# imalexlee/simple-vk-renderer

Hardware: AMD Instinct MI355X
Metric: shaded fragments/s (higher is better)
Workload: dtype f32

## Files before the change

simple-vk-renderer_amd/csrc/k_tile.hip:

```cpp
#include <hip/hip_ext.h>

#include <cstdlib>
#include <type_traits>

#include "svr_launch.h"
#include "svr_pixel.h"

namespace svr {

constexpr uint32_t REC_COMMON = 0x80000000u;
#ifndef SVR_PRIO_COST
#define SVR_PRIO_COST 200u
#endif
constexpr int BATCH = 64;
constexpr uint32_t SREC = 7;

constexpr float kG0 = 0x1.c51282p-2f, kG1 = -0x1.14a3a2p-2f, kG2 = 0x1.37536ap-3f, kG3 = -0x1.778474p-5f;

__device__ __forceinline__ float lod_from_rho2(float rho2) {
  uint32_t bits = f2u(rho2);
  int e = (int)(bits >> 23) - 127;
  float m = u2f((bits & 0x7fffffu) | 0x3f800000u);
  float t = m - 1.0f;
  float g = fmaf(fmaf(fmaf(kG3, t, kG2), t, kG1), t, kG0);
  float s = t * (1.0f - t);
  float l = fmaf(s, g, t);
  float lam = 0.5f * ((float)e + l);
  lam = (rho2 <= 0x1p+100f) ? lam : 50.0f;
  lam = (rho2 >= 0x1p-100f) ? lam : -50.0f;
  return lam;
}

__device__ __forceinline__ float lerpf(float a, float b, float t) { return fmaf(t, b - a, a); }

struct TexD {
  uint32_t base_off;
  uint32_t w, h, lw, lh, levels, filters;
  float min_lod, max_lod;
};

struct Taps {
  uint32_t o00, o10, o01, o11;
  float alpha, beta;
};
template <bool POW2 = false>
__device__ __forceinline__ Taps level_taps(int wl, int hl, uint32_t plw, uint32_t base, bool linear, float u, float v) {
  float U = (u - floorf(u)) * (float)wl;
  float V = (v - floorf(v)) * (float)hl;
  float Uh = U - 0.5f, Vh = V - 0.5f;
  float fu = floorf(linear ? Uh : U), fv = floorf(linear ? Vh : V);
  Taps tp;
  tp.alpha = linear ? Uh - fu : 0.0f;
  tp.beta = linear ? Vh - fv : 0.0f;
  int i0 = (int)fu, j0 = (int)fv;
  int i1 = linear ? i0 + 1 : i0, j1 = linear ? j0 + 1 : j0;
  if (POW2) {
    i0 &= wl - 1;
    i1 &= wl - 1;
    j0 &= hl - 1;
    j1 &= hl - 1;
  } else {
    if (i0 < 0) i0 += wl;
    if (i0 >= wl) i0 -= wl;
    if (i1 >= wl) i1 -= wl;
    if (j0 < 0) j0 += hl;
    if (j0 >= hl) j0 -= hl;
    if (j1 >= hl) j1 -= hl;
  }
  const uint32_t x0 = texel_offset_x((uint32_t)i0), x1 = texel_offset_x((uint32_t)i1);
  const uint32_t y0 = base + texel_offset_y(plw, (uint32_t)j0), y1 = base + texel_offset_y(plw, (uint32_t)j1);
  tp.o00 = y0 + x0;
  tp.o10 = y0 + x1;
  tp.o01 = y1 + x0;
  tp.o11 = y1 + x1;
  return tp;
}
__device__ __forceinline__ uint32_t texel(const uint8_t* arena, uint32_t off) {
  return *reinterpret_cast<const uint32_t*>(arena + off);
}
__device__ __forceinline__ float bilerp(uint32_t t00, uint32_t t10, uint32_t t01, uint32_t t11, int c, float a, float b) {
  return lerpf(lerpf(chan(t00, c), chan(t10, c), a), lerpf(chan(t01, c), chan(t11, c), a), b);
}

__device__ __forceinline__ float interp3(float a0, float da1, float da2, float b1, float b2, float r) {
  return fmaf(b2, da2, fmaf(b1, da1, a0)) * r;
}

struct FragAttr {
  float b1, b2, r, u, v, nx, ny, nz, light, cr, cg, cb, won;
};

__device__ __forceinline__ float quad_partner_x(float v) { return u2f((uint32_t)__builtin_amdgcn_mov_dpp((int)f2u(v), 0xB1, 0xf, 0xf, true)); }
__device__ __forceinline__ float quad_partner_y(float v) { return u2f((uint32_t)__builtin_amdgcn_mov_dpp((int)f2u(v), 0x128, 0xf, 0xf, true)); }
template <bool TRACE, bool COMMON = false, bool ATTR = false>
__device__ __forceinline__ float4 shade_pixel(const FrameParams& P, uint32_t rec, int px, int py, float* trace, const bool quads = false,
                                              FragAttr* fa = nullptr) {
  const TriRec* tr = P.recs + rec;
  const uint4* q4 = reinterpret_cast<const uint4*>(tr);
  const float4* f4 = reinterpret_cast<const float4*>(tr);
  const double2* d2 = reinterpret_cast<const double2*>(tr);
  uint4 hdr = q4[0];
  float4 zrow = f4[1];
  double2 c2 = d2[2], c3 = d2[3], c4 = d2[4], c5 = d2[5], c6 = d2[6];
  uint4 td = q4[7];
  float4 s0 = f4[8], s1 = f4[9], s2 = f4[10], s3 = f4[11], s4 = f4[12], s5 = f4[13], s6 = f4[14];
  uint32_t flags = hdr.w;
  float inv_area = zrow.w;
  double A1, B1, A2, B2, e1, e2;
  double C1 = c5.y, C2 = c6.x;
  A1 = c2.y; B1 = c4.x; A2 = c3.x; B2 = c4.y;
  double dx = (double)px, dy = (double)py;
  e1 = fma(A1, dx, fma(B1, dy, C1)) + ((flags & F_T1) ? 1.0 : 0.0);
  e2 = fma(A2, dx, fma(B2, dy, C2)) + ((flags & F_T2) ? 1.0 : 0.0);
  TexD t;
  t.base_off = (uint32_t)(unsigned long long)__double_as_longlong(c6.y);
  const uint32_t tk = (uint32_t)((unsigned long long)__double_as_longlong(c6.y) >> 32);
  t.w = td.x & 0xffffu;
  t.h = td.x >> 16;
  t.lw = td.y & 0xffu;
  t.lh = (td.y >> 8) & 0xffu;
  t.levels = (td.y >> 16) & 0xffu;
  t.filters = td.y >> 24;
  t.min_lod = u2f(td.z);
  t.max_lod = u2f(td.w);
  float b1 = (float)e1 * inv_area, b2 = (float)e2 * inv_area;
  float q0 = s0.x, dq1 = s0.y, dq2 = s0.z;
  const float qq = fmaf(b2, dq2, fmaf(b1, dq1, q0));
  float hb1 = 0.0f, hb2 = 0.0f, vb1 = 0.0f, vb2 = 0.0f, hq = 1.0f, vq = 1.0f, hr = 0.0f, vr = 0.0f;
  auto partners = [&]() {
    double sxp = (px & 1) ? -1.0 : 1.0, syp = (py & 1) ? -1.0 : 1.0;
    hb1 = (float)fma(sxp, A1, e1) * inv_area, hb2 = (float)fma(sxp, A2, e2) * inv_area;
    vb1 = (float)fma(syp, B1, e1) * inv_area, vb2 = (float)fma(syp, B2, e2) * inv_area;
    hq = fmaf(hb2, dq2, fmaf(hb1, dq1, q0)), vq = fmaf(vb2, dq2, fmaf(vb1, dq1, q0));
  };
  if (!COMMON && !quads) partners();
  const float r = COMMON ? rcp_in_window(qq) : rcp_ieee(qq);
  const uint32_t kind = COMMON ? (uint32_t)PIPE_MESH : ((flags >> F_KIND_SHIFT) & 3u);
  float cr = interp3(s1.z, s3.z, s5.z, b1, b2, r);
  float cg = interp3(s1.w, s3.w, s5.w, b1, b2, r);
  float cb = interp3(s2.x, s4.x, s6.x, b1, b2, r);
  if (ATTR) { fa->b1 = b1; fa->b2 = b2; fa->r = r; fa->won = 1.0f; }
  if (kind == PIPE_COLORED_TRIANGLE) return make_float4(cr, cg, cb, 1.0f);
  float u = interp3(s2.y, s4.y, s6.y, b1, b2, r), v = interp3(s2.z, s4.z, s6.z, b1, b2, r);
  if (ATTR) { fa->u = u; fa->v = v; }
  if (!COMMON) {
    hr = rcp_ieee(hq);
    vr = rcp_ieee(vq);
  }
  float uh, vh, uv_, vv_;
  if (quads) {
    uh = quad_partner_x(u), vh = quad_partner_x(v);
    uv_ = quad_partner_y(u), vv_ = quad_partner_y(v);
  } else {
    if (COMMON) {
      partners();
      hr = rcp_in_window(hq);
      vr = rcp_in_window(vq);
    }
    uh = interp3(s2.y, s4.y, s6.y, hb1, hb2, hr), vh = interp3(s2.z, s4.z, s6.z, hb1, hb2, hr);
    uv_ = interp3(s2.y, s4.y, s6.y, vb1, vb2, vr), vv_ = interp3(s2.z, s4.z, s6.z, vb1, vb2, vr);
  }
  float dudx = (px & 1) ? (u - uh) : (uh - u);
  float dvdx = (px & 1) ? (v - vh) : (vh - v);
  float dudy = (py & 1) ? (u - uv_) : (uv_ - u);
  float dvdy = (py & 1) ? (v - vv_) : (vv_ - v);
  float W0 = (float)t.w, H0 = (float)t.h;
  float mx = dudx * W0, my = dvdx * H0;
  float nx_ = dudy * W0, ny_ = dvdy * H0;
  float rho2 = fmaxf(fmaf(mx, mx, my * my), fmaf(nx_, nx_, ny_ * ny_));
  float lambda = fminf(fmaxf(lod_from_rho2(rho2), t.min_lod), t.max_lod);
  const bool linear = COMMON ? true : (((lambda <= 0.0f) ? (t.filters & 1u) : ((t.filters >> 1) & 1u)) != 0u);
  int q = COMMON ? (int)(tk >> 24) : (int)t.levels - 1;
  const bool mip_linear = COMMON ? true : (((t.filters >> 2) & 1u) != 0u);
  int dn = min(max((int)ceilf(lambda + 0.5f) - 1, 0), q);
  float lc = fminf(fmaxf(lambda, 0.0f), (float)q);
  float fl = floorf(lc);
  int dhi = mip_linear ? (int)fl : dn;
  float delta = mip_linear ? lc - fl : 0.0f;
  int dlo = mip_linear ? min(dhi + 1, q) : dn;
  float us = (COMMON || fabsf(u) < 8388608.0f) ? u : 0.0f, vs = (COMMON || fabsf(v) < 8388608.0f) ? v : 0.0f;
  const int whi = (int)max(t.w >> dhi, 1u), hhi = (int)max(t.h >> dhi, 1u);
  const uint32_t bhi = t.base_off + (COMMON ? packed_mip_offset(tk, (uint32_t)dhi) : mip_offset(t.lw, t.lh, (uint32_t)dhi));
  const uint32_t plw_hi = COMMON ? packed_level_lw(td.y, (uint32_t)dhi) : level_lw(t.lw, (uint32_t)dhi);
  Taps th = level_taps<COMMON>(whi, hhi, plw_hi, bhi, linear, us, vs);
  const uint8_t* tb = P.tex_arena;
  uint32_t h00 = texel(tb, th.o00), h10 = texel(tb, th.o10), h01 = texel(tb, th.o01), h11 = texel(tb, th.o11);
  const bool two_levels = __any(delta != 0.0f);
  Taps tl = th;
  uint32_t l00 = 0, l10 = 0, l01 = 0, l11 = 0;
  if (two_levels) {
    const int wlo = (int)max(t.w >> dlo, 1u), hlo = (int)max(t.h >> dlo, 1u);
    const uint32_t step = COMMON ? packed_level_bytes(tk, (uint32_t)dhi) : level_bytes(t.lw, t.lh, (uint32_t)dhi);
    const uint32_t blo = dlo != dhi ? bhi + step : bhi;
    const uint32_t plw_lo = COMMON ? packed_level_lw(td.y, (uint32_t)dlo) : level_lw(t.lw, (uint32_t)dlo);
    tl = level_taps<COMMON>(wlo, hlo, plw_lo, blo, linear, us, vs);
    l00 = texel(tb, tl.o00);
    l10 = texel(tb, tl.o10);
    l01 = texel(tb, tl.o01);
    l11 = texel(tb, tl.o11);
  }
  float4 tx;
  tx.x = bilerp(h00, h10, h01, h11, 0, th.alpha, th.beta);
  tx.y = bilerp(h00, h10, h01, h11, 1, th.alpha, th.beta);
  tx.z = bilerp(h00, h10, h01, h11, 2, th.alpha, th.beta);
  tx.w = 1.0f;
  if (two_levels) {
    tx.x = lerpf(tx.x, bilerp(l00, l10, l01, l11, 0, tl.alpha, tl.beta), delta);
    tx.y = lerpf(tx.y, bilerp(l00, l10, l01, l11, 1, tl.alpha, tl.beta), delta);
    tx.z = lerpf(tx.z, bilerp(l00, l10, l01, l11, 2, tl.alpha, tl.beta), delta);
  }
  if (TRACE) {
    trace[0] = (float)(hdr.z >> 2); trace[1] = b1; trace[2] = b2; trace[3] = r; trace[4] = u; trace[5] = v;
    trace[6] = dudx; trace[7] = dvdx; trace[8] = dudy; trace[9] = dvdy; trace[10] = lambda;
    trace[11] = tx.x; trace[12] = tx.y; trace[13] = tx.z;
    trace[26] = hb1; trace[27] = hb2; trace[28] = vb1; trace[29] = vb2; trace[30] = hr; trace[31] = vr;
  }
  if (kind == PIPE_TEX_IMAGE) {
    tx.w = bilerp(h00, h10, h01, h11, 3, th.alpha, th.beta);
    if (two_levels) tx.w = lerpf(tx.w, bilerp(l00, l10, l01, l11, 3, tl.alpha, tl.beta), delta);
    return tx;
  }
  float nx = interp3(s0.w, s2.w, s4.w, b1, b2, r);
  float ny = interp3(s1.x, s3.x, s5.x, b1, b2, r);
  float nz = interp3(s1.y, s3.y, s5.y, b1, b2, r);
  const float* L = P.scene.sunlight_direction;
  float d = fmaf(nz, L[2], fmaf(ny, L[1], nx * L[0]));
  float light = fmaxf(d, 0.1f);
  float sunw = P.scene.sunlight_color[3];
  cr = cr * tx.x;
  cg = cg * tx.y;
  cb = cb * tx.z;
  float4 o;
  o.x = fmaf(cr * light, sunw, cr * P.scene.ambient_color[0]);
  o.y = fmaf(cg * light, sunw, cg * P.scene.ambient_color[1]);
  o.z = fmaf(cb * light, sunw, cb * P.scene.ambient_color[2]);
  o.w = 1.0f;
  if (TRACE) {
    trace[15] = nx; trace[16] = ny; trace[17] = nz; trace[18] = cr; trace[19] = cg; trace[20] = cb;
    trace[21] = light; trace[22] = o.x; trace[23] = o.y; trace[24] = o.z; trace[25] = o.w;
  }
  if (ATTR) { fa->nx = nx; fa->ny = ny; fa->nz = nz; fa->light = light; fa->cr = cr; fa->cg = cg; fa->cb = cb; }
  return o;
}

template <bool INSTR, bool LIST, bool HIZ>
__device__ __forceinline__ void scan_columns(const FrameParams& P, uint4* s_cov, const uint32_t* s_list, uint32_t bin_base, uint32_t n,
                                             unsigned long long* s_depth, uint32_t* s_bm, int tx0, int ty0, int ry0, int nrows,
                                             uint32_t& n_raster, uint32_t& n_hiz_bad, uint32_t& occl) {
  auto entry = [&](uint32_t i) -> uint32_t { return LIST ? (s_list[i] & 0x7fffffffu) : P.bins[bin_base + i]; };
  const uint32_t lane = threadIdx.x & 63u, wave = threadIdx.x >> 6;
  static_assert(BATCH * 8 == 512, "two pieces per thread");
  uint4 pre0 = make_uint4(0, 0, 0, 0), pre1 = pre0;
  {
    uint32_t cnt = min((uint32_t)BATCH, n);
    const bool staged = (threadIdx.x & 7u) < SREC;
    if (staged && threadIdx.x < cnt * 8u) pre0 = reinterpret_cast<const uint4*>(P.recs + entry(threadIdx.x >> 3))[threadIdx.x & 7u];
    if (staged && threadIdx.x + 256u < cnt * 8u) pre1 = reinterpret_cast<const uint4*>(P.recs + entry(32u + (threadIdx.x >> 3)))[threadIdx.x & 7u];
  }
  constexpr uint32_t SVR_HIZ_MIN = BATCH;
  constexpr uint32_t SVR_HIZ_KEEP_COLS = 192u;
  const bool hiz = HIZ && n > (uint32_t)SVR_HIZ_MIN;
  uint32_t cur = 0, hz_cols = 0, hz_batches = 0, hz_pause = 0;
  if (hiz && threadIdx.x < 32u) s_bm[threadIdx.x] = threadIdx.x < 16u ? 0u : 0xffffffffu;
  for (uint32_t b0 = 0; b0 < n; b0 += BATCH) {
    uint32_t cnt = min((uint32_t)BATCH, n - b0);
    __syncthreads();
    const bool test = hiz && b0 && hz_pause == 0u;
    if (hiz && b0 && hz_pause) hz_pause--;
    if (test) {
      cur ^= 1u;
      const uint32_t b = threadIdx.x >> 4, k = threadIdx.x & 15u;
      const uint4* c4 = reinterpret_cast<const uint4*>(s_depth + ((b & 3u) * 8u + (k >> 1)) * TILE + (b >> 2) * 8u + (k & 1u) * 4u);
      const uint4 lo = c4[0], hi = c4[1];
// ... 79 lines not shown
          m = min(m, (by0 <= 3 && by1 >= 3) ? q.w : 0xffffffffu);
        }
        hidden = zb < m;
        if (hidden) gone = (uint32_t)cw;
        if (!INSTR && hidden) cw = 0;
      }
      if (INSTR && cw) {
        uint32_t* fl = reinterpret_cast<uint32_t*>(s_cov) + lane * SREC * 4u + 3u;
        *fl = (*fl & 0x7fffffffu) | ((hidden || (LIST && (s_list[b0 + lane] >> 31))) ? 0x80000000u : 0u);
      }
    }
    if (test) {
      const uint32_t nh = (uint32_t)__popcll(__ballot(hidden));
      hz_cols += nh + 3u * (uint32_t)__popcll(__ballot(gone >= 4u)) + 12u * (uint32_t)__popcll(__ballot(gone >= 16u));
      if (++hz_batches == 2u) {
        if (hz_cols < SVR_HIZ_KEEP_COLS) hz_pause = 6u;
        hz_cols = hz_batches = 0u;
      }
    }
    uint32_t inc = (uint32_t)cw;
#pragma unroll
    for (int off = 1; off < 64; off <<= 1) {
      uint32_t v = __shfl_up(inc, off);
      if ((int)lane >= off) inc += v;
    }
    uint32_t total = (uint32_t)__builtin_amdgcn_readlane((int)inc, 63);
    const uint32_t sh = total <= 64u ? 2u : (total <= 128u ? 1u : 0u);
    const int band_rows = nrows >> sh;
    const uint32_t items = total << sh;
    for (uint32_t c = wave; c * 64u < items; c += 4u) {
      uint32_t item = c * 64u + lane;
      uint32_t j = item >> sh, band = item & ((1u << sh) - 1u);
      bool act = item < items;
      uint32_t pos = 0;
#pragma unroll
      for (uint32_t step = 32; step >= 1; step >>= 1) {
        uint32_t v = __shfl(inc, (int)min(pos + step - 1u, 63u));
        if (pos + step <= 64u && v <= j) pos += step;
      }
      uint32_t i = min(pos, 63u);
      uint32_t excl = __shfl(inc, (int)i) - (uint32_t)__shfl(cw, (int)i);
      int col = __shfl(cx0, (int)i) + (int)(j - excl);
      if (!act) continue;
      const uint4* rec = s_cov + i * SREC;
      uint4 h = rec[0];
      int miny = (int)(int16_t)(h.x >> 16), maxy = (int)(int16_t)(h.y >> 16);
      int y0 = max(miny, ry0 + (int)band * band_rows), y1 = min(maxy, ry0 + (int)band * band_rows + band_rows - 1);
      if (y0 > y1) continue;
      uint32_t key = h.z, flags = h.w;
      float4 zr = reinterpret_cast<const float4*>(rec)[1];
      const double2* d = reinterpret_cast<const double2*>(rec);
      double2 c2 = d[2], c3 = d[3], c4 = d[4], c5 = d[5], c6 = d[6];
      double B0 = c3.y, B1 = c4.x, B2 = c4.y;
      double u1 = (flags & F_T1) ? 1.0 : 0.0, u2 = (flags & F_T2) ? 1.0 : 0.0;
      double dx = (double)col, dy = (double)y0;
      double f0 = fma(c2.x, dx, fma(B0, dy, c5.x));
      double f1 = fma(c2.y, dx, fma(B1, dy, c5.y));
      double f2 = fma(c3.x, dx, fma(B2, dy, c6.x));
      unsigned long long* cell = s_depth + (y0 - ty0) * TILE + (col - tx0);
      for (int y = y0; y <= y1; y++) {
        if (f0 >= 0.0 && f1 >= 0.0 && f2 >= 0.0) {
          if (INSTR) n_raster++;
          float b1 = (float)(f1 + u1) * zr.w, b2 = (float)(f2 + u2) * zr.w;
          float z = fmaf(b2, zr.z, fmaf(b1, zr.y, zr.x));
          z = fminf(fmaxf(z, 0.0f), 1.0f) + 0.0f;
          if (INSTR && (flags >> 31) && f2u(z) >= (uint32_t)(*cell >> 32)) n_hiz_bad++;
          atomicMax(cell, ((unsigned long long)f2u(z) << 32) | key);
        }
        f0 += B0;
        f1 += B1;
        f2 += B2;
        cell += TILE;
      }
    }
  }
}

__device__ __forceinline__ uint32_t resolve_record(const FrameParams& P, uint32_t rec, int px, int py) {
  uint4 h = *reinterpret_cast<const uint4*>(P.recs + rec);
  if ((int)(int16_t)(h.x & 0xffffu) <= (int)(int16_t)(h.y & 0xffffu)) return rec;
  double dx = (double)px, dy = (double)py;
  for (uint32_t c = 0; c < h.w; c++) {
    const TriRec* t = P.recs + h.z + c;
    if (t->minx > t->maxx || px < t->minx || px > t->maxx || py < t->miny || py > t->maxy) continue;
    if (fma(t->A[0], dx, fma(t->B[0], dy, t->C[0])) >= 0.0 && fma(t->A[1], dx, fma(t->B[1], dy, t->C[1])) >= 0.0 &&
        fma(t->A[2], dx, fma(t->B[2], dy, t->C[2])) >= 0.0)
      return h.z + c;
  }
  return rec;
}

constexpr uint32_t SORT_CAP = SPLIT_SORT_MAX;
constexpr uint32_t RANK_SORT_MAX = 1024;
#ifndef SVR_HIZ_FILTER_MIN
#define SVR_HIZ_FILTER_MIN 1024
#endif
constexpr uint32_t HIZ_AVG_ENTRIES = 96;
constexpr uint32_t HIZ_FILTER_MIN = SVR_HIZ_FILTER_MIN;
constexpr uint32_t QUARTER_LIST_CAP = 3808;
constexpr uint32_t QUEUE_CAP = 128;

template <int FMT, bool INSTR>
__device__ __forceinline__ void flush_fragments(const FrameParams& P, typename Codec<FMT>::enc_t* col, uint2* q,
                                                float4* s_src, uint32_t& qn, int tx0, int by0,
                                                uint32_t lane, uint32_t& n_shaded) {
  typedef Codec<FMT> CD;
  uint32_t cnt = min(qn, 64u);
// ... 84 lines not shown
      if (t0 < cnt) {
        if (pc < SREC) s_cov[t0 * SREC + pc] = r0;
        if (pc == 0) s_idx[t0] = ri0;
      }
      if (t0 + 32u < cnt) {
        if (pc < SREC) s_cov[(t0 + 32u) * SREC + pc] = r1;
        if (pc == 0) s_idx[t0 + 32u] = ri1;
      }
    }
    __syncthreads();
    int cx0 = 0, cw = 0;
    if (lane < cnt) {
      uint4 h = s_cov[lane * SREC];
      int minx = (int)(int16_t)(h.x & 0xffffu), miny = (int)(int16_t)(h.x >> 16);
      int maxx = (int)(int16_t)(h.y & 0xffffu), maxy = (int)(int16_t)(h.y >> 16);
      cx0 = max(minx, tx0);
      int cx1 = min(maxx, tx0 + TILE - 1);
      cw = (cx1 >= cx0 && min(maxy, by1) >= max(miny, by0)) ? cx1 - cx0 + 1 : 0;
    }
    uint32_t inc = (uint32_t)cw;
#pragma unroll
    for (int off = 1; off < 64; off <<= 1) {
      uint32_t v = __shfl_up(inc, off);
      if ((int)lane >= off) inc += v;
    }
    uint32_t total = (uint32_t)__builtin_amdgcn_readlane((int)inc, 63);
    uint32_t c = 0;
    int t = 0;
    for (;;) {
      bool full = false;
      while (c * 64u < total) {
        uint32_t j = c * 64u + lane;
        bool act = j < total;
        uint32_t pos = 0;
#pragma unroll
        for (uint32_t step = 32; step >= 1; step >>= 1) {
          uint32_t v = __shfl(inc, (int)min(pos + step - 1u, 63u));
          if (pos + step <= 64u && v <= j) pos += step;
        }
        uint32_t i = min(pos, 63u);
        uint32_t excl = __shfl(inc, (int)i) - (uint32_t)__shfl(cw, (int)i);
        int colx = __shfl(cx0, (int)i) + (int)(j - excl) - tx0;
        colx = act ? colx : 0;
        const uint4* rec = s_cov + i * SREC;
        uint4 h = rec[0];
        int y0 = (int)(int16_t)(h.x >> 16), y1 = (int)(int16_t)(h.y >> 16);
        uint32_t flags = h.w, ri = s_idx[i];
        float4 zr = reinterpret_cast<const float4*>(rec)[1];
        const double2* d = reinterpret_cast<const double2*>(rec);
        double2 c2 = d[2], c3 = d[3], c4 = d[4], c5 = d[5], c6 = d[6];
        double B0 = c3.y, B1 = c4.x, B2 = c4.y;
        double dx = (double)(tx0 + colx), dy = (double)(by0 + t);
        double f0 = fma(c2.x, dx, fma(B0, dy, c5.x));
        const double u1 = (flags & F_T1) ? 1.0 : 0.0, u2 = (flags & F_T2) ? 1.0 : 0.0;
        double g1 = fma(c2.y, dx, fma(B1, dy, c5.y));
        double g2 = fma(c3.x, dx, fma(B2, dy, c6.x));
#pragma unroll 1
        for (; t < rpw; t++) {
          int y = by0 + t;
          bool inside = act && y >= y0 && y <= y1 && f0 >= 0.0 && g1 >= 0.0 && g2 >= 0.0;
          if (INSTR) n_raster += inside ? 1u : 0u;
          float b1 = (float)(g1 + u1) * zr.w, b2 = (float)(g2 + u2) * zr.w;
          float z = fmaf(b2, zr.z, fmaf(b1, zr.y, zr.x));
          z = fminf(fmaxf(z, 0.0f), 1.0f) + 0.0f;
          bool pass = inside && f2u(z) >= s_z[(y - ty0) * TILE + colx];
          unsigned long long m = __ballot(pass);
          f0 += B0;
          g1 += B1;
          g2 += B2;
          if (m) {
            if (pass) q[qn + (uint32_t)__popcll(m & below)] = make_uint2((uint32_t)(t * TILE + colx), ri | ((h.z & 2u) ? REC_COMMON : 0u));
            qn += (uint32_t)__popcll(m);
            if (qn >= 64u) {
              full = true;
              t++;
              break;
            }
          }
        }
        if (full) break;
        t = 0;
        c++;
      }
      if (!full) break;
      flush_fragments<FMT, INSTR>(P, col, q, s_src, qn, tx0, by0, lane, n_shaded);
      if (t == rpw) {
        t = 0;
        c++;
      }
    }
  }
  while (qn) flush_fragments<FMT, INSTR>(P, col, q, s_src, qn, tx0, by0, lane, n_shaded);
}

template <uint32_t K, typename KeyT>
__device__ __forceinline__ void count_ranks(const KeyT* s, uint32_t n, const KeyT (&mine)[K], uint32_t (&rank)[K]) {
#pragma unroll
  for (uint32_t k = 0; k < K; k++) rank[k] = 0;
  for (uint32_t j = 0; j < n; j++) {
    KeyT v = s[j];
#pragma unroll
    for (uint32_t k = 0; k < K; k++) rank[k] += v < mine[k] ? 1u : 0u;
  }
}

template <uint32_t K>
__device__ __forceinline__ void rank_sort(const FrameParams& P, unsigned char* lds, uint32_t bin_base, uint32_t n, uint32_t* out, const uint32_t wv) {
// ... 932 lines not shown
```

simple-vk-renderer_amd/csrc/svr_api.hip:

```cpp
#include <algorithm>
#include <chrono>
#include <cmath>
#include <cstdio>
#include <numeric>

#include "svr_context.h"
#include "svr_cull.h"

using namespace svr;

namespace {
thread_local std::string g_err;
}
int svr::fail(int code, const std::string& msg) {
  g_err = msg;
  return code;
}
int svr::hip_fail(hipError_t e, const char* what) {
  return fail(e == hipErrorOutOfMemory ? SVR_ERR_OUT_OF_MEMORY : SVR_ERR_DEVICE, std::string(what) + ": " + hipGetErrorString(e));
}

namespace {

uint16_t host_f32_to_f16(float f) {
  uint32_t x;
  std::memcpy(&x, &f, 4);
  uint32_t sign = (x >> 16) & 0x8000u, ax = x & 0x7fffffffu;
  if (ax >= 0x7f800000u) return (uint16_t)(sign | (ax > 0x7f800000u ? 0x7e00u : 0x7c00u));
  if (ax >= 0x477ff000u) return (uint16_t)(sign | 0x7c00u);
  if (ax >= 0x38800000u) {
    uint32_t mant = ax & 0x7fffffu, h = (((ax >> 23) - 112) << 10) | (mant >> 13), rem = mant & 0x1fffu;
    if (rem > 0x1000u || (rem == 0x1000u && (h & 1u))) h++;
    return (uint16_t)(sign | h);
  }
  if (ax < 0x33000000u) return (uint16_t)sign;
  uint32_t mant = (ax & 0x7fffffu) | 0x800000u;
  int shift = 126 - (int)(ax >> 23);
  uint32_t h = mant >> shift, rem = mant & ((1u << shift) - 1u), half = 1u << (shift - 1);
  if (rem > half || (rem == half && (h & 1u))) h++;
  return (uint16_t)(sign | h);
}

MeshRes* get_mesh(SvrContext* ctx, SvrMesh h) {
  if (h == 0 || h > ctx->meshes.size() || !ctx->meshes[h - 1].alive) return nullptr;
  return &ctx->meshes[h - 1];
}
ImageRes* get_image(SvrContext* ctx, SvrImage h) {
  if (h == 0 || h > ctx->images.size() || !ctx->images[h - 1].alive) return nullptr;
  return &ctx->images[h - 1];
}

TexBinding make_binding(const ImageRes& im, const SvrSamplerDesc& s) {
  TexBinding tb;
  std::memset(&tb, 0, sizeof(tb));
  uint32_t filters = (uint32_t)s.mag_filter | ((uint32_t)s.min_filter << 1) | ((uint32_t)s.mipmap_mode << 2);
  tb.base_off = im.arena_off;
  tb.pad0 = tex_consts(im.lw, im.lh, im.levels);
  tb.wh = im.w | (im.h << 16);
  tb.info = im.lw | (im.lh << 8) | (im.levels << 16) | (filters << 24);
  tb.min_lod = s.min_lod;
  tb.max_lod = s.max_lod;
  return tb;
}

constexpr size_t ARENA_MAX = (size_t)0xffffff00u;
constexpr size_t ARENA_ALIGN = 256;

int arena_alloc(SvrContext* ctx, size_t bytes, uint32_t* off) {
  bytes = (bytes + ARENA_ALIGN - 1) & ~(ARENA_ALIGN - 1);
  for (size_t i = 0; i < ctx->tex_holes.size(); i++) {
    auto& h = ctx->tex_holes[i];
    if (h.second >= bytes) {
      *off = (uint32_t)h.first;
      h.first += bytes;
      h.second -= bytes;
      if (h.second == 0) ctx->tex_holes.erase(ctx->tex_holes.begin() + (long)i);
      return SVR_OK;
    }
  }
  if (ctx->tex_arena_top + bytes > ARENA_MAX)
    return fail(SVR_ERR_OUT_OF_MEMORY, "svr_create_image: more than 4 GiB of texels in one context");
  if (ctx->tex_arena_top + bytes > ctx->tex_arena_cap) {
    size_t want = std::max(ctx->tex_arena_cap * 2, ctx->tex_arena_top + bytes);
    want = std::min(ARENA_MAX, (want + ((size_t)64 << 20) - 1) & ~(((size_t)64 << 20) - 1));
    if (int e = finish_pending(ctx)) return e;
    HIPCHK(hipStreamSynchronize(ctx->stream));
    DevPtr<uint8_t> grown;
    DEV_ALLOC(grown, want);
    if (ctx->tex_arena_top) {
      hipError_t r = hipMemcpy(grown.get(), ctx->tex_arena.get(), ctx->tex_arena_top, hipMemcpyDeviceToDevice);
      if (r != hipSuccess) return fail(SVR_ERR_DEVICE, std::string("hipMemcpy(texel arena): ") + hipGetErrorString(r));
    }
    ctx->tex_arena = std::move(grown);
    ctx->tex_arena_cap = want;
  }
  *off = (uint32_t)ctx->tex_arena_top;
  ctx->tex_arena_top += bytes;
  return SVR_OK;
}

void arena_free(SvrContext* ctx, size_t off, size_t bytes) {
  bytes = (bytes + ARENA_ALIGN - 1) & ~(ARENA_ALIGN - 1);
  auto& holes = ctx->tex_holes;
  size_t i = 0;
  while (i < holes.size() && holes[i].first < off) i++;
  holes.insert(holes.begin() + (long)i, std::make_pair(off, bytes));
  if (i + 1 < holes.size() && holes[i].first + holes[i].second == holes[i + 1].first) {
    holes[i].second += holes[i + 1].second;
    holes.erase(holes.begin() + (long)i + 1);
  }
  if (i > 0 && holes[i - 1].first + holes[i - 1].second == holes[i].first) {
    holes[i - 1].second += holes[i].second;
    holes.erase(holes.begin() + (long)i);
// ... 1413 lines not shown
```

simple-vk-renderer_amd/csrc/svr_device.h:

```cpp
#pragma once

#include <hip/hip_runtime.h>
#include <stdint.h>

#include "../../include/svr.h"

namespace svr {

constexpr int TILE = 32;
constexpr int TILE_SHIFT = 5;
constexpr int WAVE = 64;
constexpr float GUARD = 16384.0f;
constexpr uint32_t NO_REC = 0xffffffffu;
#ifndef SVR_RCP_VARIANT
#define SVR_RCP_VARIANT 1
#endif

enum PipelineKind : uint32_t { PIPE_MESH = 0, PIPE_COLORED_TRIANGLE = 1, PIPE_TEX_IMAGE = 2 };

constexpr uint32_t F_T1 = 1u;
constexpr uint32_t F_T2 = 2u;
constexpr uint32_t F_KIND_SHIFT = 4;
constexpr uint32_t F_TRANSPARENT = 256u;
constexpr uint32_t F_VIEW_SHIFT = 24;
// ... 59 lines not shown
  float min_lod, max_lod;
  uint32_t pad[2];
};
static_assert(sizeof(TexBinding) == 32, "TexBinding layout");

constexpr uint32_t TEX_TILE_LW = 3, TEX_TILE_LH = 2;
constexpr uint32_t TEX_TILE_BYTES = 4u << (TEX_TILE_LW + TEX_TILE_LH);
__host__ __device__ inline uint32_t level_lw(uint32_t lw, uint32_t level) { return lw > level + TEX_TILE_LW ? lw - level : TEX_TILE_LW; }
__host__ __device__ inline uint32_t level_lh(uint32_t lh, uint32_t level) { return lh > level + TEX_TILE_LH ? lh - level : TEX_TILE_LH; }
__host__ __device__ inline uint32_t level_bytes(uint32_t lw, uint32_t lh, uint32_t level) { return 4u << (level_lw(lw, level) + level_lh(lh, level)); }

__host__ __device__ inline uint32_t mip_offset(uint32_t lw, uint32_t lh, uint32_t level) {
  const uint32_t cw = level_lw(lw, 0), ch = level_lh(lh, 0), nw = cw - TEX_TILE_LW, nh = ch - TEX_TILE_LH;
  const uint32_t a = nw < nh ? nw : nh, b = nw < nh ? nh : nw;
  const uint32_t l1 = level < a ? level : a, l2 = level < b ? level : b;
  const uint32_t ones = l1 ? (0x55555555u >> (32u - 2u * l1)) : 0u;
  uint32_t off = ones << ((cw + ch + 4u - 2u * l1) & 31u);
  if (level > a) off += (8u << (cw + ch - 2u * a)) - (8u << (cw + ch - a - l2));
  if (level > b) off += (level - b) * TEX_TILE_BYTES;
  return off;
}
__host__ __device__ inline uint32_t texel_offset_x(uint32_t x) {
  return ((x >> TEX_TILE_LW) << (TEX_TILE_LW + TEX_TILE_LH + 2u)) | ((x & ((1u << TEX_TILE_LW) - 1u)) << 2u);
}
__host__ __device__ inline uint32_t texel_offset_y(uint32_t plw, uint32_t y) {
  return ((y >> TEX_TILE_LH) << (plw + TEX_TILE_LH + 2u)) | ((y & ((1u << TEX_TILE_LH) - 1u)) << (TEX_TILE_LW + 2u));
}
__host__ __device__ inline uint32_t texel_offset(uint32_t plw, uint32_t x, uint32_t y) { return texel_offset_x(x) + texel_offset_y(plw, y); }

__host__ __device__ inline uint32_t tex_consts(uint32_t lw, uint32_t lh, uint32_t levels) {
  const uint32_t cw = level_lw(lw, 0), ch = level_lh(lh, 0), nw = cw - TEX_TILE_LW, nh = ch - TEX_TILE_LH;
  return (nw < nh ? nw : nh) | ((nw < nh ? nh : nw) << 8) | ((cw + ch) << 16) | ((levels ? levels - 1u : 0u) << 24);
}
__host__ __device__ inline uint32_t packed_level_lw(uint32_t info, uint32_t level) {
  const int d = (int)(info & 0xffu) - (int)level;
  return (uint32_t)(d > (int)TEX_TILE_LW ? d : (int)TEX_TILE_LW);
}
__host__ __device__ inline uint32_t packed_level_lh(uint32_t info, uint32_t level) {
  const int d = (int)((info >> 8) & 0xffu) - (int)level;
  return (uint32_t)(d > (int)TEX_TILE_LH ? d : (int)TEX_TILE_LH);
}
__host__ __device__ inline uint32_t packed_level_bytes(uint32_t k, uint32_t level) {
  const uint32_t a = k & 0xffu, b = (k >> 8) & 0xffu, cc = (k >> 16) & 0xffu;
  return 4u << (cc - (level < a ? level : a) - (level < b ? level : b));
}
__host__ __device__ inline uint32_t packed_mip_offset(uint32_t k, uint32_t level) {
  const uint32_t a = k & 0xffu, b = (k >> 8) & 0xffu, cc = (k >> 16) & 0xffu;
  const uint32_t l1 = level < a ? level : a, l2 = level < b ? level : b;
  uint32_t off = (0x2aaaaaaau >> (31u - 2u * l1)) << ((cc + 4u - 2u * l1) & 31u);
  if (level > a) off += (8u << (cc - 2u * a)) - (8u << (cc - a - l2));
  if (level > b) off += (level - b) * TEX_TILE_BYTES;
  return off;
}

__host__ __device__ inline bool frag_ranges_ok(float q0, float dq1, float dq2, double A1, double B1, double A2, double B2, float inv_area,
                                               const float (&uv)[6]) {
  const float fa1 = (float)A1, fb1 = (float)B1, fa2 = (float)A2, fb2 = (float)B2;
  const float gx = (fa1 * dq1 + fa2 * dq2) * inv_area, gy = (fb1 * dq1 + fb2 * dq2) * inv_area;
  const float a1 = fa1 < 0.0f ? -fa1 : fa1, b1 = fb1 < 0.0f ? -fb1 : fb1, a2 = fa2 < 0.0f ? -fa2 : fa2, b2 = fb2 < 0.0f ? -fb2 : fb2;
  const float steps = ((a1 > b1 ? a1 : b1) * (dq1 < 0.0f ? -dq1 : dq1) + (a2 > b2 ? a2 : b2) * (dq2 < 0.0f ? -dq2 : dq2)) * inv_area;
  const float q1 = q0 + dq1, q2 = q0 + dq2;
  const float lo0 = q0 < q1 ? (q0 < q2 ? q0 : q2) : (q1 < q2 ? q1 : q2), hi0 = q0 > q1 ? (q0 > q2 ? q0 : q2) : (q1 > q2 ? q1 : q2);
  const float ax = gx < 0.0f ? -gx : gx, ay = gy < 0.0f ? -gy : gy, G = ax > ay ? ax : ay;
  const float mag = steps + (q0 < 0.0f ? -q0 : q0) + (dq1 < 0.0f ? -dq1 : dq1) + (dq2 < 0.0f ? -dq2 : dq2);
  const float allow = mag * 0x1p-19f + 0x1p-100f;
  const float lo = lo0 - G - allow, hi = hi0 + G + allow;
  float sum = 0.0f;
  for (int i = 0; i < 6; i++) sum += uv[i] < 0.0f ? -uv[i] : uv[i];
  return lo >= 0x1p-94f && hi <= 0x1p95f && mag <= 0x1p100f && sum * (lo + 0x1p-18f * hi) < 4194304.0f * lo;
}

struct TriRec {
  int16_t minx, miny, maxx, maxy;
  uint32_t key;
  uint32_t flags;
  float z0, dz1, dz2, inv_area;
  double A[3], B[3], C[3];
  uint32_t tex_off, tex_pad;
  uint32_t tex_wh, tex_info;
  float tex_min_lod, tex_max_lod;
  float q0, dq1, dq2;
  float a0[8], da1[8], da2[8];
  float pad2;
  uint32_t object, primitive;
  float pad3[2];
};
static_assert(sizeof(TriRec) == 256, "TriRec layout");
static_assert(offsetof(TriRec, object) == 240, "TriRec layout: the ID words are piece 15's x and y");
constexpr uint32_t REC_ID_PIECE = offsetof(TriRec, object) / 16u;
static_assert(offsetof(TriRec, A) == 32 && offsetof(TriRec, tex_off) == 104 && offsetof(TriRec, tex_wh) == 112 &&
                  offsetof(TriRec, q0) == 128, "TriRec layout");

struct ClipItem {
  uint32_t draw;
  uint32_t tri;
};

struct Counters {
  uint32_t n_clip;
  uint32_t n_extra;
  uint32_t total_entries;
  uint32_t overflow;
  unsigned long long rasterized;
  unsigned long long shaded;
  unsigned long long binned;
  uint32_t n_big;
// ... 394 lines not shown
```

simple-vk-renderer_amd/csrc/svr_pixel.h:

```cpp
#pragma once

#include <hip/hip_fp16.h>

#include "svr_device.h"

namespace svr {

__device__ __forceinline__ float pin(float x) {
  asm volatile("" : "+v"(x));
  return x;
}
__device__ __forceinline__ uint32_t h16(float x) { return __half_as_ushort(__float2half_rn(pin(x))); }
__device__ __forceinline__ float half_bits_to_float(uint32_t h) { return __half2float(__ushort_as_half((unsigned short)h)); }

constexpr float HALF_MAX = 65504.0f;
__device__ __forceinline__ float san(float v) { return v > 0.0f ? (v < HALF_MAX ? v : HALF_MAX) : 0.0f; }

constexpr float kInv255 = 0x1.010102p-8f;
__device__ __forceinline__ uint32_t un8(float f) { return (uint32_t)__float2int_rn(fminf(fmaxf(f, 0.0f), 1.0f) * 255.0f); }
__device__ __forceinline__ float chan(uint32_t t, int c) { return (float)((t >> (8 * c)) & 0xffu) * kInv255; }

template <int FMT>
struct Codec;
template <>
struct Codec<SVR_COLOR_RGBA16F> {
  typedef uint2 enc_t;
  static __device__ __forceinline__ enc_t encode(float4 c) {
    c.x = pin(c.x); c.y = pin(c.y); c.z = pin(c.z); c.w = pin(c.w);
    uint32_t r = __half_as_ushort(__float2half_rn(c.x)), g = __half_as_ushort(__float2half_rn(c.y));
    uint32_t b = __half_as_ushort(__float2half_rn(c.z)), a = __half_as_ushort(__float2half_rn(c.w));
    return make_uint2(r | (g << 16), b | (a << 16));
  }
  static __device__ __forceinline__ float4 decode(enc_t e) {
    return make_float4(half_bits_to_float(e.x & 0xffffu), half_bits_to_float(e.x >> 16), half_bits_to_float(e.y & 0xffffu),
                       half_bits_to_float(e.y >> 16));
  }
};
template <>
struct Codec<SVR_COLOR_RGBA8> {
  typedef uint32_t enc_t;
  static __device__ __forceinline__ enc_t encode(float4 c) { return un8(c.x) | (un8(c.y) << 8) | (un8(c.z) << 16) | (un8(c.w) << 24); }
  static __device__ __forceinline__ float4 decode(enc_t e) { return make_float4(chan(e, 0), chan(e, 1), chan(e, 2), chan(e, 3)); }
};

__device__ __forceinline__ bool aligned_to(const void* p, uintptr_t n) { return (reinterpret_cast<uintptr_t>(p) & (n - 1u)) == 0u; }
__device__ __forceinline__ uint32_t clamp_to(int v, uint32_t n) { return v < 0 ? 0u : ((uint32_t)v > n - 1u ? n - 1u : (uint32_t)v); }

}
```

Baseline: 46.89 billion.

## Specialize common-path texture sampling with exponent scaling, med3 clamps and packed f16 encode

Adds a dedicated common-path texture sampler that uses ldexp with power-of-two masks in place of multiplies and width/height shifts. It also uses fmed3 for the LOD clamps, sign-bit flips in place of double FMAs for partner barycentrics, and a branchless top-left bias. Separately, the RGBA16F encoder now does packed two-wide half conversion, and the host clamps min_lod to max_lod so the med3 clamp stays valid. These are many small instruction-count reductions in the hot per-fragment shading path, with some risk of numerical differences from changed rounding.

```diff
diff --git a/simple-vk-renderer_amd/csrc/k_tile.hip b/simple-vk-renderer_amd/csrc/k_tile.hip
--- a/simple-vk-renderer_amd/csrc/k_tile.hip
+++ b/simple-vk-renderer_amd/csrc/k_tile.hip
@@ -32,6 +32,8 @@
 }
 
 __device__ __forceinline__ float lerpf(float a, float b, float t) { return fmaf(t, b - a, a); }
+__device__ __forceinline__ float clamp_med3(float x, float lo, float hi) { return __builtin_amdgcn_fmed3f(x, lo, hi); }
+__device__ __forceinline__ double top_left_bias(uint32_t flags, uint32_t bit) { return (double)((flags / bit) & 1u); }
 
 struct TexD {
   uint32_t base_off;
@@ -43,7 +45,6 @@
   uint32_t o00, o10, o01, o11;
   float alpha, beta;
 };
-template <bool POW2 = false>
 __device__ __forceinline__ Taps level_taps(int wl, int hl, uint32_t plw, uint32_t base, bool linear, float u, float v) {
   float U = (u - floorf(u)) * (float)wl;
   float V = (v - floorf(v)) * (float)hl;
@@ -54,19 +55,12 @@
   tp.beta = linear ? Vh - fv : 0.0f;
   int i0 = (int)fu, j0 = (int)fv;
   int i1 = linear ? i0 + 1 : i0, j1 = linear ? j0 + 1 : j0;
-  if (POW2) {
-    i0 &= wl - 1;
-    i1 &= wl - 1;
-    j0 &= hl - 1;
-    j1 &= hl - 1;
-  } else {
-    if (i0 < 0) i0 += wl;
-    if (i0 >= wl) i0 -= wl;
-    if (i1 >= wl) i1 -= wl;
-    if (j0 < 0) j0 += hl;
-    if (j0 >= hl) j0 -= hl;
-    if (j1 >= hl) j1 -= hl;
-  }
+  if (i0 < 0) i0 += wl;
+  if (i0 >= wl) i0 -= wl;
+  if (i1 >= wl) i1 -= wl;
+  if (j0 < 0) j0 += hl;
+  if (j0 >= hl) j0 -= hl;
+  if (j1 >= hl) j1 -= hl;
   const uint32_t x0 = texel_offset_x((uint32_t)i0), x1 = texel_offset_x((uint32_t)i1);
   const uint32_t y0 = base + texel_offset_y(plw, (uint32_t)j0), y1 = base + texel_offset_y(plw, (uint32_t)j1);
   tp.o00 = y0 + x0;
@@ -75,11 +69,57 @@
   tp.o11 = y1 + x1;
   return tp;
 }
+__device__ __forceinline__ Taps level_taps_exp(int kw, int kh, uint32_t plw, uint32_t base, float u, float v) {
+  float U = ldexpf(u - floorf(u), kw);
+  float V = ldexpf(v - floorf(v), kh);
+  float Uh = U - 0.5f, Vh = V - 0.5f;
+  float fu = floorf(Uh), fv = floorf(Vh);
+  Taps tp;
+  tp.alpha = Uh - fu;
+  tp.beta = Vh - fv;
+  const int i0 = (int)fu, j0 = (int)fv;
+  const uint32_t mw = (1u << kw) - 1u, mh = (1u << kh) - 1u;
+  const uint32_t x0 = texel_offset_x((uint32_t)i0 & mw), x1 = texel_offset_x((uint32_t)(i0 + 1) & mw);
+  const uint32_t y0 = base + texel_offset_y(plw, (uint32_t)j0 & mh), y1 = base + texel_offset_y(plw, (uint32_t)(j0 + 1) & mh);
+  tp.o00 = y0 + x0;
+  tp.o10 = y0 + x1;
+  tp.o01 = y1 + x0;
+  tp.o11 = y1 + x1;
+  return tp;
+}
 __device__ __forceinline__ uint32_t texel(const uint8_t* arena, uint32_t off) {
   return *reinterpret_cast<const uint32_t*>(arena + off);
 }
 __device__ __forceinline__ float bilerp(uint32_t t00, uint32_t t10, uint32_t t01, uint32_t t11, int c, float a, float b) {
   return lerpf(lerpf(chan(t00, c), chan(t10, c), a), lerpf(chan(t01, c), chan(t11, c), a), b);
+}
+
+__device__ __forceinline__ float4 common_texture(const uint8_t* tb, uint32_t base_off, uint32_t tk, uint32_t info, int dhi, int dlo,
+                                                 float delta, float u, float v) {
+  const uint32_t lw = info & 0xffu, lh = (info >> 8) & 0xffu;
+  auto kexp = [](uint32_t l, int d) { return (int)__builtin_elementwise_sub_sat(l, (uint32_t)d); };
+  const uint32_t bhi = base_off + packed_mip_offset(tk, (uint32_t)dhi);
+  const Taps th = level_taps_exp(kexp(lw, dhi), kexp(lh, dhi), packed_level_lw(info, (uint32_t)dhi), bhi, u, v);
+  const uint32_t h00 = texel(tb, th.o00), h10 = texel(tb, th.o10), h01 = texel(tb, th.o01), h11 = texel(tb, th.o11);
+  float4 tx;
+  tx.w = 1.0f;
+  const bool two_levels = __any(delta != 0.0f);
+  Taps tl = th;
+  uint32_t l00 = 0, l10 = 0, l01 = 0, l11 = 0;
+  if (two_levels) {
+    const uint32_t blo = dlo != dhi ? bhi + packed_level_bytes(tk, (uint32_t)dhi) : bhi;
+    tl = level_taps_exp(kexp(lw, dlo), kexp(lh, dlo), packed_level_lw(info, (uint32_t)dlo), blo, u, v);
+    l00 = texel(tb, tl.o00), l10 = texel(tb, tl.o10), l01 = texel(tb, tl.o01), l11 = texel(tb, tl.o11);
+  }
+  tx.x = bilerp(h00, h10, h01, h11, 0, th.alpha, th.beta);
+  tx.y = bilerp(h00, h10, h01, h11, 1, th.alpha, th.beta);
+  tx.z = bilerp(h00, h10, h01, h11, 2, th.alpha, th.beta);
+  if (two_levels) {
+    tx.x = lerpf(tx.x, bilerp(l00, l10, l01, l11, 0, tl.alpha, tl.beta), delta);
+    tx.y = lerpf(tx.y, bilerp(l00, l10, l01, l11, 1, tl.alpha, tl.beta), delta);
+    tx.z = lerpf(tx.z, bilerp(l00, l10, l01, l11, 2, tl.alpha, tl.beta), delta);
+  }
+  return tx;
 }
 
 __device__ __forceinline__ float interp3(float a0, float da1, float da2, float b1, float b2, float r) {
@@ -110,8 +150,8 @@
   double C1 = c5.y, C2 = c6.x;
   A1 = c2.y; B1 = c4.x; A2 = c3.x; B2 = c4.y;
   double dx = (double)px, dy = (double)py;
-  e1 = fma(A1, dx, fma(B1, dy, C1)) + ((flags & F_T1) ? 1.0 : 0.0);
-  e2 = fma(A2, dx, fma(B2, dy, C2)) + ((flags & F_T2) ? 1.0 : 0.0);
+  e1 = fma(A1, dx, fma(B1, dy, C1)) + top_left_bias(flags, F_T1);
+  e2 = fma(A2, dx, fma(B2, dy, C2)) + top_left_bias(flags, F_T2);
   TexD t;
   t.base_off = (uint32_t)(unsigned long long)__double_as_longlong(c6.y);
   const uint32_t tk = (uint32_t)((unsigned long long)__double_as_longlong(c6.y) >> 32);
@@ -128,9 +168,16 @@
   const float qq = fmaf(b2, dq2, fmaf(b1, dq1, q0));
   float hb1 = 0.0f, hb2 = 0.0f, vb1 = 0.0f, vb2 = 0.0f, hq = 1.0f, vq = 1.0f, hr = 0.0f, vr = 0.0f;
   auto partners = [&]() {
-    double sxp = (px & 1) ? -1.0 : 1.0, syp = (py & 1) ? -1.0 : 1.0;
-    hb1 = (float)fma(sxp, A1, e1) * inv_area, hb2 = (float)fma(sxp, A2, e2) * inv_area;
-    vb1 = (float)fma(syp, B1, e1) * inv_area, vb2 = (float)fma(syp, B2, e2) * inv_area;
+    if (COMMON) {
+      const int sx = (int)((uint32_t)px << 31), sy = (int)((uint32_t)py << 31);
+      auto flip = [](double a, int s) { return __hiloint2double(__double2hiint(a) ^ s, __double2loint(a)); };
+      hb1 = (float)(e1 + flip(A1, sx)) * inv_area, hb2 = (float)(e2 + flip(A2, sx)) * inv_area;
+      vb1 = (float)(e1 + flip(B1, sy)) * inv_area, vb2 = (float)(e2 + flip(B2, sy)) * inv_area;
+    } else {
+      double sxp = (px & 1) ? -1.0 : 1.0, syp = (py & 1) ? -1.0 : 1.0;
+      hb1 = (float)fma(sxp, A1, e1) * inv_area, hb2 = (float)fma(sxp, A2, e2) * inv_area;
+      vb1 = (float)fma(syp, B1, e1) * inv_area, vb2 = (float)fma(syp, B2, e2) * inv_area;
+    }
     hq = fmaf(hb2, dq2, fmaf(hb1, dq1, q0)), vq = fmaf(vb2, dq2, fmaf(vb1, dq1, q0));
   };
   if (!COMMON && !quads) partners();
@@ -160,65 +207,69 @@
     uh = interp3(s2.y, s4.y, s6.y, hb1, hb2, hr), vh = interp3(s2.z, s4.z, s6.z, hb1, hb2, hr);
     uv_ = interp3(s2.y, s4.y, s6.y, vb1, vb2, vr), vv_ = interp3(s2.z, s4.z, s6.z, vb1, vb2, vr);
   }
-  float dudx = (px & 1) ? (u - uh) : (uh - u);
-  float dvdx = (px & 1) ? (v - vh) : (vh - v);
-  float dudy = (py & 1) ? (u - uv_) : (uv_ - u);
-  float dvdy = (py & 1) ? (v - vv_) : (vv_ - v);
+  float dudx = (COMMON || !(px & 1)) ? (uh - u) : (u - uh);
+  float dvdx = (COMMON || !(px & 1)) ? (vh - v) : (v - vh);
+  float dudy = (COMMON || !(py & 1)) ? (uv_ - u) : (u - uv_);
+  float dvdy = (COMMON || !(py & 1)) ? (vv_ - v) : (v - vv_);
   float W0 = (float)t.w, H0 = (float)t.h;
-  float mx = dudx * W0, my = dvdx * H0;
-  float nx_ = dudy * W0, ny_ = dvdy * H0;
+  float mx = COMMON ? ldexpf(dudx, (int)t.lw) : dudx * W0, my = COMMON ? ldexpf(dvdx, (int)t.lh) : dvdx * H0;
+  float nx_ = COMMON ? ldexpf(dudy, (int)t.lw) : dudy * W0, ny_ = COMMON ? ldexpf(dvdy, (int)t.lh) : dvdy * H0;
   float rho2 = fmaxf(fmaf(mx, mx, my * my), fmaf(nx_, nx_, ny_ * ny_));
-  float lambda = fminf(fmaxf(lod_from_rho2(rho2), t.min_lod), t.max_lod);
+  float lambda = COMMON ? clamp_med3(lod_from_rho2(rho2), t.min_lod, t.max_lod) : fminf(fmaxf(lod_from_rho2(rho2), t.min_lod), t.max_lod);
   const bool linear = COMMON ? true : (((lambda <= 0.0f) ? (t.filters & 1u) : ((t.filters >> 1) & 1u)) != 0u);
   int q = COMMON ? (int)(tk >> 24) : (int)t.levels - 1;
   const bool mip_linear = COMMON ? true : (((t.filters >> 2) & 1u) != 0u);
   int dn = min(max((int)ceilf(lambda + 0.5f) - 1, 0), q);
-  float lc = fminf(fmaxf(lambda, 0.0f), (float)q);
+  float lc = COMMON ? clamp_med3(lambda, 0.0f, (float)q) : fminf(fmaxf(lambda, 0.0f), (float)q);
   float fl = floorf(lc);
   int dhi = mip_linear ? (int)fl : dn;
   float delta = mip_linear ? lc - fl : 0.0f;
   int dlo = mip_linear ? min(dhi + 1, q) : dn;
   float us = (COMMON || fabsf(u) < 8388608.0f) ? u : 0.0f, vs = (COMMON || fabsf(v) < 8388608.0f) ? v : 0.0f;
-  const int whi = (int)max(t.w >> dhi, 1u), hhi = (int)max(t.h >> dhi, 1u);
-  const uint32_t bhi = t.base_off + (COMMON ? packed_mip_offset(tk, (uint32_t)dhi) : mip_offset(t.lw, t.lh, (uint32_t)dhi));
-  const uint32_t plw_hi = COMMON ? packed_level_lw(td.y, (uint32_t)dhi) : level_lw(t.lw, (uint32_t)dhi);
-  Taps th = level_taps<COMMON>(whi, hhi, plw_hi, bhi, linear, us, vs);
-  const uint8_t* tb = P.tex_arena;
-  uint32_t h00 = texel(tb, th.o00), h10 = texel(tb, th.o10), h01 = texel(tb, th.o01), h11 = texel(tb, th.o11);
-  const bool two_levels = __any(delta != 0.0f);
-  Taps tl = th;
-  uint32_t l00 = 0, l10 = 0, l01 = 0, l11 = 0;
-  if (two_levels) {
-    const int wlo = (int)max(t.w >> dlo, 1u), hlo = (int)max(t.h >> dlo, 1u);
-    const uint32_t step = COMMON ? packed_level_bytes(tk, (uint32_t)dhi) : level_bytes(t.lw, t.lh, (uint32_t)dhi);
-    const uint32_t blo = dlo != dhi ? bhi + step : bhi;
-    const uint32_t plw_lo = COMMON ? packed_level_lw(td.y, (uint32_t)dlo) : level_lw(t.lw, (uint32_t)dlo);
-    tl = level_taps<COMMON>(wlo, hlo, plw_lo, blo, linear, us, vs);
-    l00 = texel(tb, tl.o00);
-    l10 = texel(tb, tl.o10);
-    l01 = texel(tb, tl.o01);
-    l11 = texel(tb, tl.o11);
-  }
   float4 tx;
-  tx.x = bilerp(h00, h10, h01, h11, 0, th.alpha, th.beta);
-  tx.y = bilerp(h00, h10, h01, h11, 1, th.alpha, th.beta);
-  tx.z = bilerp(h00, h10, h01, h11, 2, th.alpha, th.beta);
-  tx.w = 1.0f;
-  if (two_levels) {
-    tx.x = lerpf(tx.x, bilerp(l00, l10, l01, l11, 0, tl.alpha, tl.beta), delta);
-    tx.y = lerpf(tx.y, bilerp(l00, l10, l01, l11, 1, tl.alpha, tl.beta), delta);
-    tx.z = lerpf(tx.z, bilerp(l00, l10, l01, l11, 2, tl.alpha, tl.beta), delta);
-  }
-  if (TRACE) {
-    trace[0] = (float)(hdr.z >> 2); trace[1] = b1; trace[2] = b2; trace[3] = r; trace[4] = u; trace[5] = v;
-    trace[6] = dudx; trace[7] = dvdx; trace[8] = dudy; trace[9] = dvdy; trace[10] = lambda;
-    trace[11] = tx.x; trace[12] = tx.y; trace[13] = tx.z;
-    trace[26] = hb1; trace[27] = hb2; trace[28] = vb1; trace[29] = vb2; trace[30] = hr; trace[31] = vr;
-  }
-  if (kind == PIPE_TEX_IMAGE) {
-    tx.w = bilerp(h00, h10, h01, h11, 3, th.alpha, th.beta);
-    if (two_levels) tx.w = lerpf(tx.w, bilerp(l00, l10, l01, l11, 3, tl.alpha, tl.beta), delta);
-    return tx;
+  if constexpr (COMMON) {
+    tx = common_texture(P.tex_arena, t.base_off, tk, td.y, dhi, dlo, delta, us, vs);
+  } else {
+    const int whi = (int)max(t.w >> dhi, 1u), hhi = (int)max(t.h >> dhi, 1u);
+    const uint32_t bhi = t.base_off + mip_offset(t.lw, t.lh, (uint32_t)dhi);
+    const uint32_t plw_hi = level_lw(t.lw, (uint32_t)dhi);
+    Taps th = level_taps(whi, hhi, plw_hi, bhi, linear, us, vs);
+    const uint8_t* tb = P.tex_arena;
+    uint32_t h00 = texel(tb, th.o00), h10 = texel(tb, th.o10), h01 = texel(tb, th.o01), h11 = texel(tb, th.o11);
+    const bool two_levels = __any(delta != 0.0f);
+    Taps tl = th;
+    uint32_t l00 = 0, l10 = 0, l01 = 0, l11 = 0;
+    if (two_levels) {
+      const int wlo = (int)max(t.w >> dlo, 1u), hlo = (int)max(t.h >> dlo, 1u);
+      const uint32_t step = level_bytes(t.lw, t.lh, (uint32_t)dhi);
+      const uint32_t blo = dlo != dhi ? bhi + step : bhi;
+      const uint32_t plw_lo = level_lw(t.lw, (uint32_t)dlo);
+      tl = level_taps(wlo, hlo, plw_lo, blo, linear, us, vs);
+      l00 = texel(tb, tl.o00);
+      l10 = texel(tb, tl.o10);
+      l01 = texel(tb, tl.o01);
+      l11 = texel(tb, tl.o11);
+    }
+    tx.x = bilerp(h00, h10, h01, h11, 0, th.alpha, th.beta);
+    tx.y = bilerp(h00, h10, h01, h11, 1, th.alpha, th.beta);
+    tx.z = bilerp(h00, h10, h01, h11, 2, th.alpha, th.beta);
+    tx.w = 1.0f;
+    if (two_levels) {
+      tx.x = lerpf(tx.x, bilerp(l00, l10, l01, l11, 0, tl.alpha, tl.beta), delta);
+      tx.y = lerpf(tx.y, bilerp(l00, l10, l01, l11, 1, tl.alpha, tl.beta), delta);
+      tx.z = lerpf(tx.z, bilerp(l00, l10, l01, l11, 2, tl.alpha, tl.beta), delta);
+    }
+    if (TRACE) {
+      trace[0] = (float)(hdr.z >> 2); trace[1] = b1; trace[2] = b2; trace[3] = r; trace[4] = u; trace[5] = v;
+      trace[6] = dudx; trace[7] = dvdx; trace[8] = dudy; trace[9] = dvdy; trace[10] = lambda;
+      trace[11] = tx.x; trace[12] = tx.y; trace[13] = tx.z;
+      trace[26] = hb1; trace[27] = hb2; trace[28] = vb1; trace[29] = vb2; trace[30] = hr; trace[31] = vr;
+    }
+    if (kind == PIPE_TEX_IMAGE) {
+      tx.w = bilerp(h00, h10, h01, h11, 3, th.alpha, th.beta);
+      if (two_levels) tx.w = lerpf(tx.w, bilerp(l00, l10, l01, l11, 3, tl.alpha, tl.beta), delta);
+      return tx;
+    }
   }
   float nx = interp3(s0.w, s2.w, s4.w, b1, b2, r);
   float ny = interp3(s1.x, s3.x, s5.x, b1, b2, r);
@@ -404,7 +455,7 @@
       const double2* d = reinterpret_cast<const double2*>(rec);
       double2 c2 = d[2], c3 = d[3], c4 = d[4], c5 = d[5], c6 = d[6];
       double B0 = c3.y, B1 = c4.x, B2 = c4.y;
-      double u1 = (flags & F_T1) ? 1.0 : 0.0, u2 = (flags & F_T2) ? 1.0 : 0.0;
+      double u1 = top_left_bias(flags, F_T1), u2 = top_left_bias(flags, F_T2);
       double dx = (double)col, dy = (double)y0;
       double f0 = fma(c2.x, dx, fma(B0, dy, c5.x));
       double f1 = fma(c2.y, dx, fma(B1, dy, c5.y));
@@ -595,7 +646,7 @@
         double B0 = c3.y, B1 = c4.x, B2 = c4.y;
         double dx = (double)(tx0 + colx), dy = (double)(by0 + t);
         double f0 = fma(c2.x, dx, fma(B0, dy, c5.x));
-        const double u1 = (flags & F_T1) ? 1.0 : 0.0, u2 = (flags & F_T2) ? 1.0 : 0.0;
+        const double u1 = top_left_bias(flags, F_T1), u2 = top_left_bias(flags, F_T2);
         double g1 = fma(c2.y, dx, fma(B1, dy, c5.y));
         double g2 = fma(c3.x, dx, fma(B2, dy, c6.x));
 #pragma unroll 1
diff --git a/simple-vk-renderer_amd/csrc/svr_api.hip b/simple-vk-renderer_amd/csrc/svr_api.hip
--- a/simple-vk-renderer_amd/csrc/svr_api.hip
+++ b/simple-vk-renderer_amd/csrc/svr_api.hip
@@ -58,7 +58,7 @@
   tb.pad0 = tex_consts(im.lw, im.lh, im.levels);
   tb.wh = im.w | (im.h << 16);
   tb.info = im.lw | (im.lh << 8) | (im.levels << 16) | (filters << 24);
-  tb.min_lod = s.min_lod;
+  tb.min_lod = binding_min_lod(s.min_lod, s.max_lod);
   tb.max_lod = s.max_lod;
   return tb;
 }
diff --git a/simple-vk-renderer_amd/csrc/svr_device.h b/simple-vk-renderer_amd/csrc/svr_device.h
--- a/simple-vk-renderer_amd/csrc/svr_device.h
+++ b/simple-vk-renderer_amd/csrc/svr_device.h
@@ -135,6 +135,8 @@
   if (level > b) off += (level - b) * TEX_TILE_BYTES;
   return off;
 }
+
+__host__ __device__ inline float binding_min_lod(float lo, float hi) { return lo <= hi ? lo : hi; }
 
 __host__ __device__ inline bool frag_ranges_ok(float q0, float dq1, float dq2, double A1, double B1, double A2, double B2, float inv_area,
                                                const float (&uv)[6]) {
diff --git a/simple-vk-renderer_amd/csrc/svr_pixel.h b/simple-vk-renderer_amd/csrc/svr_pixel.h
--- a/simple-vk-renderer_amd/csrc/svr_pixel.h
+++ b/simple-vk-renderer_amd/csrc/svr_pixel.h
@@ -26,10 +26,11 @@
 struct Codec<SVR_COLOR_RGBA16F> {
   typedef uint2 enc_t;
   static __device__ __forceinline__ enc_t encode(float4 c) {
+    typedef float f32x2 __attribute__((ext_vector_type(2)));
+    typedef _Float16 f16x2 __attribute__((ext_vector_type(2)));
     c.x = pin(c.x); c.y = pin(c.y); c.z = pin(c.z); c.w = pin(c.w);
-    uint32_t r = __half_as_ushort(__float2half_rn(c.x)), g = __half_as_ushort(__float2half_rn(c.y));
-    uint32_t b = __half_as_ushort(__float2half_rn(c.z)), a = __half_as_ushort(__float2half_rn(c.w));
-    return make_uint2(r | (g << 16), b | (a << 16));
+    const f16x2 rg = __builtin_convertvector((f32x2){c.x, c.y}, f16x2), ba = __builtin_convertvector((f32x2){c.z, c.w}, f16x2);
+    return make_uint2(__builtin_bit_cast(uint32_t, rg), __builtin_bit_cast(uint32_t, ba));
   }
   static __device__ __forceinline__ float4 decode(enc_t e) {
     return make_float4(half_bits_to_float(e.x & 0xffffu), half_bits_to_float(e.x >> 16), half_bits_to_float(e.y & 0xffffu),
```

Result: faster. 48.27 billion, median of 6 (+2.9%).
